# ocrickard/piper-swift

Hardware: AMD Instinct MI355X
Metric: audio-sec/wall-sec (RTF^-1) with ms/utterance, Piper VITS en_GB-medium geometry, scale-bench factor (higher is better)
Workload: dtype f32; 1 GPU; medium factor=8: 112 ids, 336 frames, 86016 samples (3.901 s audio) per utterance, 1 utterance per step per GPU; factor=8, phoneme_count=112, frames=336, samples=86016, parallelism=utterance-replicas x1 (one-shot RCCL weight broadcast)

## Files before the change

### piper-swift_amd/csrc/conv.h

```cpp
#pragma once
#include "common.h"

namespace ph {

enum Prologue : int {
  PRO_NONE = 0,
  PRO_LRELU = 1,
  PRO_AVG3_LRELU = 2,
  PRO_LN = 3,
};

enum Epilogue : int {
  EPI_STORE = 0,
  EPI_RELU = 1,
  EPI_TANH = 2,
  EPI_RSUB = 3,
  EPI_WN_RES_SKIP = 4,
  EPI_WN_SKIP_LAST = 5,
  EPI_CONVT = 6,
  EPI_MRF_MEAN = 7,
};

struct ConvArgs {
  const float* x = nullptr;
// ... 1 lines not shown
  const float* x3 = nullptr;
  const float* w = nullptr;
  const float* w16 = nullptr;
  const float* w8 = nullptr;
  const float* w16g = nullptr;
  const float* bias = nullptr;
  const float* res = nullptr;
  const float* skip = nullptr;
  float* y = nullptr;
  float* y2 = nullptr;
  int N = 1, Cin = 0, Cout = 0, K = 1, dil = 1, padL = 0, Lin = 0, Lout = 0;
  int stride = 1, groups = 1;
  int64_t x_batch_stride = 0;
  int64_t y_batch_stride = 0;
  int64_t y2_batch_stride = 0;
  int in_ch_base = 0, in_ch_sign = 1;
  int out_ch_base = 0, out_ch_sign = 1;
  int y_len = 0;
  int prologue = PRO_NONE;
  float alpha = 0.0f;
  int epilogue = EPI_STORE;
  int gate = 0;
  unsigned long long* trace = nullptr;
  int wn_c = 0;
  int ct_stride = 0, ct_padL = 0, ct_Lout = 0;
  int ct_shift = -1;
  const float* mrf_a = nullptr;
  const float* mrf_b = nullptr;
  float alpha2 = 0.0f;
  const int* len_ptr = nullptr;
  int len_mul = 1;
  float* stats_out = nullptr;
  const float* ln_stats = nullptr;
  const float* ln_gamma = nullptr;
  const float* ln_beta = nullptr;
  float* ln_out = nullptr;
  float ln_eps = 1e-5f;
  int ln_self = 0;
};

size_t packed_conv_floats(int Cout, int Cin, int K, int tm = 32);
size_t packed_convt_floats(int Cin, int Cout, int K, int s, int tm = 32);
int pack_conv_weights(hipStream_t s, const float* w, int Cout, int Cin, int K, float* packed, int tm = 32);
int pack_convt_weights(hipStream_t s, const float* w, int Cin, int Cout, int K, int stride, float* packed, int tm = 32);
int pack_conv_weights_gate16(hipStream_t s, const float* w, int Cout, int Cin, int K, float* packed);
size_t packed_conv_rows8_floats(int Cout, int Cin, int K);
int pack_conv_weights_rows8(hipStream_t s, const float* w, int Cout, int Cin, int K, float* packed);
int conv_pick_tile(piper_hip_ctx* ctx, int Cout, int Lout, int N, int gate);

bool conv_mfma_eligible(int Cout, int Cin, int K, int stride, int groups);
int launch_conv_mfma(piper_hip_ctx* ctx, hipStream_t s, const ConvArgs& a);
int try_launch_conv_lean(piper_hip_ctx* ctx, hipStream_t s, const ConvArgs& a);
bool conv_lean_ln_self_ok(piper_hip_ctx* ctx, int Cin, int Cout, int K, int padL, int L, int N);
int try_launch_conv_short(piper_hip_ctx* ctx, hipStream_t s, const ConvArgs& a);
int launch_conv_direct(piper_hip_ctx* ctx, hipStream_t s, const ConvArgs& a);
int launch_convt_direct(piper_hip_ctx* ctx, hipStream_t s, const float* x, const float* w, const float* bias, float* y, int N,
                        int Cin, int Lin, int Cout, int K, int stride, int dil, int padL, int Lout, int groups);

inline double conv_flops(int Cout, int Cin_per_g, int K, int64_t Lout) { return 2.0 * Cout * (double)Lout * Cin_per_g * K; }

}
```

### piper-swift_amd/csrc/conv_lean.hip

```cpp
#include "conv.h"

namespace ph {
namespace {

typedef float f32x4 __attribute__((ext_vector_type(4)));

struct LeanArgs {
  const float *x, *w, *bias, *res, *skip;
  float *y, *y2;
  const int* len_ptr;
  int len_mul, Lin, Lout, Cout, y_len, nsteps, wn_c;
  int x_row_bytes;
  int x_base_bytes;
  int q_stride;
  int kk_sign;
  int out_ch_base, out_ch_sign;
  int x_batch_bytes;
  long long x_bs, y_bs, y2_bs;
};

__device__ __forceinline__ float bload(__amdgpu_buffer_rsrc_t r, int voff, int soff) {
  return __builtin_bit_cast(float, __builtin_amdgcn_raw_buffer_load_b32(r, voff, soff, 0));
}

// ... 13 lines not shown
  const int soff0 = a.x_base_bytes + wave * NQ * a.q_stride;
  float av[NQ], bv[NQ];
#pragma unroll
  for (int i = 0; i < NQ; i++) av[i] = wa[i * 64];
  {
    const int voff = vrow + min(ch * 16 + j, a.Lin - 1) * 4;
#pragma unroll
    for (int i = 0; i < NQ; i++) bv[i] = bload(rx, voff, soff0 + i * a.q_stride);
  }
  const int row = 16 * mt + 4 * kk + wave;
  const float bias = (wave < 4 && a.bias) ? a.bias[min(row, a.Cout - 1)] : 0.0f;
  for (int it = 0;; it++) {
    const int t0 = ch * 16;
    const int nxt = ch + (int)gridDim.y;
    const bool more = nxt < nch && nxt * 16 < lim;
    f32x4 acc = {0.0f, 0.0f, 0.0f, 0.0f};
#pragma unroll
    for (int i = 0; i < NQ; i++) acc = __builtin_amdgcn_mfma_f32_16x16x4f32(av[i], bv[i], acc, 0, 0, 0);
    if (more) {
      const int voff = vrow + min(nxt * 16 + j, a.Lin - 1) * 4;
#pragma unroll
      for (int i = 0; i < NQ; i++) bv[i] = bload(rx, voff, soff0 + i * a.q_stride);
    }
    float* red = red_all + (it & 1) * (8 * 4 * 64);
#pragma unroll
    for (int r = 0; r < 4; r++) red[(wave * 4 + r) * 64 + lane] = acc[r];
    __syncthreads();
    if (wave < 4) {
      const int col = t0 + j;
      float v = bias;
      float part[8];
#pragma unroll
      for (int s = 0; s < 8; s++) part[s] = red[(s * 4 + wave) * 64 + lane];
#pragma unroll
      for (int s = 0; s < 8; s++) v += part[s];
      if (row < a.Cout && col < a.Lout) {
        if constexpr (MODE == EPI_STORE) {
          const long long idx = (long long)n * a.y_bs + (a.out_ch_base + a.out_ch_sign * row) * a.y_len + col;
          a.y[idx] = a.res ? v + a.res[idx] : v;
        } else if constexpr (MODE == EPI_RSUB) {
          const long long idx = (long long)n * a.y_bs + (a.out_ch_base + a.out_ch_sign * row) * a.y_len + col;
          a.y[idx] = a.res[idx] - v;
        } else if constexpr (MODE == EPI_WN_RES_SKIP) {
          if (row < a.wn_c) {
            const long long idx = (long long)n * a.y_bs + row * a.y_len + col;
            a.y[idx] = a.res[idx] + v;
          } else {
            const long long idx = (long long)n * a.y2_bs + (row - a.wn_c) * a.y_len + col;
            a.y2[idx] = (a.skip ? a.skip[idx] : 0.0f) + v;
          }
        } else {
          const long long idx = (long long)n * a.y2_bs + row * a.y_len + col;
          a.y2[idx] = (a.skip ? a.skip[idx] : 0.0f) + v;
        }
      }
    }
    if (!more) break;
    ch = nxt;
  }
}

struct GateArgs {
  const float *x, *w, *bias;
  float* y;
  const int* len_ptr;
  int len_mul, Lin, Lout, rows_out, y_len, nsteps, pad, x_batch_bytes;
  long long x_bs, y_bs;
};

template <int K, int NQ>
__global__ __launch_bounds__(512) void conv_gate_kernel(const GateArgs a, const int nch) {
  constexpr int W = 16 + K - 1, PITCH = (W + 3) & ~3, ROWS = 4 * NQ, NS = NQ * K;
  constexpr int NLB = (ROWS + 15) / 16;
  constexpr int OOB = 0x7fffffff;
  static_assert(K - 1 <= 4, "halo piece is four columns wide");
  __shared__ float xs_all[8 * ROWS * PITCH];
  __shared__ float red_all[2 * 8 * 4 * 64];
  const int lane = threadIdx.x & 63;
  const int wave = __builtin_amdgcn_readfirstlane((int)(threadIdx.x >> 6));
  const int mt = blockIdx.x, n = blockIdx.z;
  const int Lv = a.len_ptr ? min(a.len_ptr[n] * a.len_mul, a.Lin) : a.Lin;
  int ch = blockIdx.y;
  if (ch * 16 >= Lv) return;
  const int j = lane & 15, kk = lane >> 4;
  const __amdgpu_buffer_rsrc_t rx = __builtin_amdgcn_make_buffer_rsrc((void*)(a.x + (long long)n * a.x_bs), 0, a.x_batch_bytes, 0x00020000);
  const float* wa = a.w + (((long long)mt * a.nsteps + wave * NS) << 6) + lane;
  float av[NS];
#pragma unroll
  for (int s = 0; s < NS; s++) av[s] = wa[s * 64];
  const int rB = lane >> 2, cB = 16 + (lane & 3);
  const int sbase = wave * ROWS * a.Lin * 4;
  float xa[NQ], xb[NLB];
  auto request = [&](int t0) {
    const int posA = t0 - a.pad + j;
    const int voffA = (posA >= 0 && posA < Lv) ? (kk * a.Lin + posA) * 4 : OOB;
    const int posB = t0 - a.pad + cB;
    const int voffB = ((lane & 3) < K - 1 && posB >= 0 && posB < Lv) ? (rB * a.Lin + posB) * 4 : OOB;
#pragma unroll
    for (int i = 0; i < NQ; i++) xa[i] = bload(rx, voffA, sbase + i * 16 * a.Lin);
#pragma unroll
    for (int i = 0; i < NLB; i++) xb[i] = bload(rx, (rB + 16 * i < ROWS) ? voffB : OOB, sbase + i * 64 * a.Lin);
  };
  request(ch * 16);
  float* xs = xs_all + wave * (ROWS * PITCH);
  const float* xw = xs + kk * PITCH + j;
  const int i8 = 4 * kk + wave;
// ... 395 lines not shown
  }
  if (c.K == 3 && c.w8 && c.Cin == 768 && c.prologue == PRO_NONE && c.epilogue == EPI_STORE && !c.stats_out && !c.gate && c.dil == 1 && c.padL == 1 &&
      c.Lin == c.Lout && c.in_ch_sign == 1 && c.in_ch_base == 0 && c.out_ch_sign == 1 && c.out_ch_base == 0 && c.N <= 65535) {
    const int mt8 = (int)ceil_div(c.Cout, 8), nch = (int)ceil_div(c.Lout, 16);
    if ((int64_t)mt8 * nch * c.N <= 2 * (int64_t)ctx->num_cus && nch <= 65535 && c.x_batch_stride * 4 < 0x7fffffffLL) {
      LeanArgs a;
      a.x = c.x; a.w = c.w8; a.bias = c.bias; a.res = c.res; a.skip = nullptr; a.y = c.y; a.y2 = nullptr;
      a.len_ptr = c.len_ptr; a.len_mul = c.len_mul;
      a.Lin = c.Lin; a.Lout = c.Lout; a.Cout = c.Cout; a.y_len = c.y_len; a.wn_c = 0; a.nsteps = (c.Cin / 4) * c.K;
      a.x_row_bytes = c.Lin * 4; a.kk_sign = 1; a.x_base_bytes = 0; a.q_stride = 16 * c.Lin; a.out_ch_base = 0; a.out_ch_sign = 1;
      a.x_batch_bytes = (int)(c.x_batch_stride * 4); a.x_bs = c.x_batch_stride; a.y_bs = c.y_batch_stride; a.y2_bs = 0;
      const int w_bytes = mt8 * a.nsteps * 128;
      constexpr int NQ = 24;
      const size_t lds = (size_t)(8 * 4 * 64 + 8 * (4 * NQ) * 20) * sizeof(float);
      static bool configured[kMaxDevices] = {};
      if (lds_optin_needed(configured))
        (void)hipFuncSetAttribute((const void*)conv_k3_r8_kernel<NQ>, hipFuncAttributeMaxDynamicSharedMemorySize, 160 * 1024);
      hipLaunchKernelGGL((conv_k3_r8_kernel<NQ>), dim3((unsigned)mt8, (unsigned)nch, (unsigned)c.N), dim3(512), lds, s, a, w_bytes);
      hipError_t e = hipGetLastError();
      if (e != hipSuccess) PH_FAIL(PIPER_HIP_ERR_LAUNCH, "conv_lean (8-row tiles) launch failed: %s", hipGetErrorString(e));
      return 1;
    }
  }
  if (c.K != 1 || c.prologue != PRO_NONE || c.stats_out || !c.w16) return 0;
  if (c.epilogue != EPI_STORE && c.epilogue != EPI_RSUB && c.epilogue != EPI_WN_RES_SKIP && c.epilogue != EPI_WN_SKIP_LAST) return 0;
  if ((c.epilogue == EPI_RSUB || c.epilogue == EPI_WN_RES_SKIP) && !c.res) return 0;
  if (c.Cin % 32 || c.padL != 0 || c.Lin != c.Lout || c.N > 65535 || c.Lout < 1) return 0;
  const int NQ = c.Cin / 32;
  if (NQ != 3 && NQ != 6) return 0;
  if (c.in_ch_sign != 1 && c.in_ch_sign != -1) return 0;
  const int mtiles = (int)ceil_div(c.Cout, 16), nchunks = (int)ceil_div(c.Lout, 16);
  if ((int64_t)mtiles * nchunks * c.N > 64 * (int64_t)ctx->num_cus) return 0;
  if (c.x_batch_stride * 4 >= 0x7fffffffLL) return 0;
  LeanArgs a;
  a.x = c.x; a.w = c.w16; a.bias = c.bias; a.res = c.res; a.skip = c.skip; a.y = c.y; a.y2 = c.y2;
  a.len_ptr = c.len_ptr; a.len_mul = c.len_mul;
  a.Lin = c.Lin; a.Lout = c.Lout; a.Cout = c.Cout; a.y_len = c.y_len; a.wn_c = c.wn_c;
  a.nsteps = c.Cin / 4;
  a.x_row_bytes = c.Lin * 4;
  a.kk_sign = c.in_ch_sign;
  a.x_base_bytes = (c.in_ch_sign > 0 ? c.in_ch_base : c.in_ch_base - 3) * c.Lin * 4;
  a.q_stride = c.in_ch_sign * 16 * c.Lin;
  a.out_ch_base = c.out_ch_base; a.out_ch_sign = c.out_ch_sign;
  a.x_batch_bytes = (int)(c.x_batch_stride * 4);
  a.x_bs = c.x_batch_stride; a.y_bs = c.y_batch_stride; a.y2_bs = c.y2_batch_stride;
  const dim3 grid((unsigned)mtiles, (unsigned)chunk_groups(ctx, mtiles, nchunks, c.N), (unsigned)c.N);
  const bool ok = NQ == 3 ? launch_lean_nq<3>(s, grid, a, c.epilogue, nchunks) : launch_lean_nq<6>(s, grid, a, c.epilogue, nchunks);
  if (!ok) return 0;
  hipError_t e = hipGetLastError();
  if (e != hipSuccess) PH_FAIL(PIPER_HIP_ERR_LAUNCH, "conv_lean launch failed: %s", hipGetErrorString(e));
  return 1;
}

}
namespace ph { namespace { PH_WARM(conv_lean, (conv_k1_kernel<6, 0>)); } }
```

### piper-swift_amd/csrc/voice.hip

```cpp
#include <algorithm>
#include <cmath>
#include <cstdlib>
#include <chrono>
#include <functional>
#include <memory>

#include "../../include/piper_hip_voice_layout.h"
#include "conv.h"
#include "conv_bf16.h"
#include "conv_win.h"
#include "rng.h"

namespace ph {
int validate_config(const piper_hip_voice_config* c);
int launch_rel_attention(piper_hip_ctx* ctx, hipStream_t s, const float* q, const float* k, const float* v, const float* ek,
                         const float* ev, float* out, int N, int H, int d, int T, int w, int64_t in_batch_stride,
                         int64_t out_batch_stride, const int* len_ptr);
int rel_attention_split_parts(piper_hip_ctx* ctx, int N, int H, int d, int T, int w);
int launch_rel_attention_split(piper_hip_ctx* ctx, hipStream_t s, const float* q, const float* k, const float* v, const float* ek,
                               const float* ev, float* out, int N, int H, int d, int T, int w, int64_t in_batch_stride,
                               int64_t out_batch_stride, const int* len_ptr, int nsplit, float* part_o, float* part_ml);
size_t dp_scalars_bytes(int n);
void dp_scalars_fill(void* host, int i, float noise_w, float length_scale, unsigned gen, unsigned seed);
bool flow_seam_eligible(int H, int half);
// ... 174 lines not shown
  hipEvent_t ev_in = nullptr;
  float* stats = nullptr;
  std::vector<void*> owned;
  int64_t* ids = nullptr;
  int32_t* frame2id = nullptr;
  float* noise = nullptr;
  float* noise_scale = nullptr;
  unsigned* rng = nullptr;
  float* audio = nullptr;
  int64_t n_samples = 0;
  std::vector<Step> steps;
  struct Tap {
    const float* p;
    int C, row, unit;
    size_t batch_stride;
  };
  std::map<std::string, Tap> taps;
  hipGraph_t graph = nullptr;
  hipGraphExec_t exec = nullptr;
  bool timed = false;
  bool parallel = false;
  float* zin = nullptr;
  const float* z_out = nullptr;
  hipGraph_t front_graph = nullptr;
  hipGraphExec_t front_exec = nullptr;
  int st_chunk = 0, st_next = -1, st_halo = 0;
  int bs_n = 0;
  std::vector<int> bs_next;
  std::vector<uint8_t> bs_dropped;
  int* bs_desc = nullptr;
  float* bs_pack = nullptr;
  size_t bs_pack_cap = 0;
};

}

struct piper_hip_voice {
  piper_hip_ctx* ctx = nullptr;
  piper_hip_voice_config cfg{};
  float* blob = nullptr;
  float* packed = nullptr;
  size_t blob_floats = 0, packed_floats = 0;
  std::map<std::string, piper_tensor_desc> index;
  struct EncLayer {
    ConvW qkv, o, f1, f2;
    const float *ek, *ev, *g1, *b1, *g2, *b2;
    float* qkv_bias;
  };
  std::vector<EncLayer> enc;
  ConvW proj;
  struct Coupling {
    ConvW pre, post;
    std::vector<ConvW> in, rs;
  };
  std::vector<Coupling> flows;
  ConvW conv_pre, conv_post;
  struct DdsLayer {
    const float *dw_w, *dw_b, *g1, *b1, *g2, *b2;
    ConvW pw;
  };
  struct DpBlock {
    int flow = 0;
    ConvW pre, proj;
    std::vector<DdsLayer> dds;
  };
  std::vector<DpBlock> dp;
  const float *dp_m = nullptr, *dp_logs = nullptr;
  struct Stage {
    ConvW up;
    int Cin, Cout, K, stride, pad;
    std::vector<std::vector<ConvW>> rb;
  };
  std::vector<Stage> stages;
  struct ConvWB {
    const uint16_t* w = nullptr;
    const float* bias = nullptr;
    int Cout = 0, Cin = 0, K = 0;
  };
  int precision = PIPER_HIP_PRECISION_F32;
  ConvWB conv_pre_b;
  std::vector<ConvWB> up_b;
  std::vector<std::vector<std::vector<ConvWB>>> rb_b;
  std::vector<void*> owned;
  std::vector<std::unique_ptr<Slot>> plans;
  std::vector<StreamSet> free_sets;
  double last_build_ms[6] = {0, 0, 0, 0, 0, 0};
  size_t plan_cache_max = 128, plan_cache_bytes = (size_t)24 << 30;
  struct Staging {
    int64_t* h_ids = nullptr; int32_t* h_f2i = nullptr; int* h_lens = nullptr; float* h_audio = nullptr;
    size_t cap_t = 0, cap_f = 0, cap_lens = 0, audio_cap = 0;
    char* h_misc = nullptr; float* h_dpn = nullptr; int32_t* h_res = nullptr;
    size_t cap_misc = 0, cap_dpn = 0, cap_res = 0;
    float* h_noise = nullptr;
    size_t cap_noise = 0;
    int* h_desc = nullptr;
    size_t cap_desc = 0;
    std::vector<hipEvent_t> chunk_ev;
  } staging[kMaxSlots];
  Slot* attached[kMaxSlots] = {};
  Slot* attached_dp[kMaxSlots] = {};
  uint64_t use_clock = 0;
  int hop = 1;
};

namespace {

// ... 62 lines not shown
  const piper_hip_voice_config& c = v->cfg;
  const int H = c.hidden, I = c.inter;
  char nm[128];
  v->enc.clear(); v->flows.clear(); v->stages.clear();
  for (int l = 0; l < c.n_layers; l++) {
    piper_hip_voice::EncLayer L{};
    L.qkv_bias = qkv_bias ? (*qkv_bias)[l] : nullptr;
    L.qkv.Cout = 3 * H; L.qkv.Cin = H; L.qkv.K = 1; L.qkv.mfma = true;
    float* p = pk.take(3 * packed_conv_floats(H, H, 1));
    float* p16 = pk.take(3 * packed_conv_floats(H, H, 1, 16));
    L.qkv.w = p;
    L.qkv.w16 = p16;
    if (!dry) {
      static const char* qkv[3] = {"conv_q", "conv_k", "conv_v"};
      for (int j = 0; j < 3; j++) {
        snprintf(nm, sizeof nm, "enc_p.encoder.attn_layers.%d.%s", l, qkv[j]);
        pack_conv_weights(pk.s, tensor(v, std::string(nm) + ".weight"), H, H, 1, p + j * packed_conv_floats(H, H, 1));
        pack_conv_weights(pk.s, tensor(v, std::string(nm) + ".weight"), H, H, 1, p16 + j * packed_conv_floats(H, H, 1, 16), 16);
        PH_HIP(hipMemcpyAsync(L.qkv_bias + j * H, tensor(v, std::string(nm) + ".bias"), H * sizeof(float),
                              hipMemcpyDeviceToDevice, pk.s), PIPER_HIP_ERR_LAUNCH);
      }
      L.qkv.bias = L.qkv_bias;
    }
    snprintf(nm, sizeof nm, "enc_p.encoder.attn_layers.%d.conv_o", l);
    L.o = make_conv(pk, dry, nm, H, H, 1);
    snprintf(nm, sizeof nm, "enc_p.encoder.ffn_layers.%d.conv_1", l);
    L.f1 = make_conv(pk, dry, nm, c.ffn, H, c.ffn_kernel);
    snprintf(nm, sizeof nm, "enc_p.encoder.ffn_layers.%d.conv_2", l);
    L.f2 = make_conv(pk, dry, nm, H, c.ffn, c.ffn_kernel, true, false, false, true);
    if (!dry) {
      snprintf(nm, sizeof nm, "enc_p.encoder.attn_layers.%d.emb_rel_k", l); L.ek = tensor(v, nm);
      snprintf(nm, sizeof nm, "enc_p.encoder.attn_layers.%d.emb_rel_v", l); L.ev = tensor(v, nm);
      snprintf(nm, sizeof nm, "enc_p.encoder.norm_layers_1.%d.gamma", l); L.g1 = tensor(v, nm);
      snprintf(nm, sizeof nm, "enc_p.encoder.norm_layers_1.%d.beta", l); L.b1 = tensor(v, nm);
      snprintf(nm, sizeof nm, "enc_p.encoder.norm_layers_2.%d.gamma", l); L.g2 = tensor(v, nm);
      snprintf(nm, sizeof nm, "enc_p.encoder.norm_layers_2.%d.beta", l); L.b2 = tensor(v, nm);
    }
    v->enc.push_back(L);
  }
  v->proj = make_conv(pk, dry, "enc_p.proj", 2 * I, H, 1);
  for (int f = 0; f < c.n_flows; f++) {
    piper_hip_voice::Coupling C;
    snprintf(nm, sizeof nm, "flow.flows.%d.pre", 2 * f);
    C.pre = make_conv(pk, dry, nm, H, I / 2, 1);
    for (int i = 0; i < c.wn_layers; i++) {
      snprintf(nm, sizeof nm, "flow.flows.%d.enc.in_layers.%d", 2 * f, i);
      C.in.push_back(make_conv(pk, dry, nm, 2 * H, H, c.wn_kernel, true, false, true));
      snprintf(nm, sizeof nm, "flow.flows.%d.enc.res_skip_layers.%d", 2 * f, i);
      C.rs.push_back(make_conv(pk, dry, nm, (i + 1 < c.wn_layers) ? 2 * H : H, H, 1));
    }
    snprintf(nm, sizeof nm, "flow.flows.%d.post", 2 * f);
    C.post = make_conv(pk, dry, nm, I / 2, H, 1);
    v->flows.push_back(C);
  }
  v->conv_pre = make_conv(pk, dry, "dec.conv_pre", c.up_initial, I, 7);
  int ch = c.up_initial;
  for (int u = 0; u < c.n_ups; u++) {
    piper_hip_voice::Stage S;
    S.Cin = ch; S.Cout = ch / 2; S.K = c.up_kernels[u]; S.stride = c.up_rates[u]; S.pad = (S.K - S.stride) / 2;
    const int J = (S.K + S.stride - 1) / S.stride;
    S.up.Cout = S.Cout * S.stride; S.up.Cin = S.Cin; S.up.K = J; S.up.mfma = true;
    float* p = pk.take(packed_convt_floats(S.Cin, S.Cout, S.K, S.stride));
    float* p16 = pk.take(packed_convt_floats(S.Cin, S.Cout, S.K, S.stride, 16));
    S.up.w = p;
    S.up.w16 = p16;
    const bool ct_win = convt_win_eligible(S.Cin, S.Cout, S.K, S.stride, S.pad, 4);
    float* p4 = ct_win ? pk.take(packed_convt_win_floats(S.Cin, S.Cout, S.K, S.stride)) : nullptr;
    S.up.w4 = ct_win ? p4 : nullptr;
    const bool ct_pipe = convt_pipe_eligible(S.Cin, S.Cout, S.K, S.stride, S.pad, 4);
    float* p5 = ct_pipe ? pk.take(packed_convt_pipe_floats(S.Cin, S.Cout, S.K, S.stride)) : nullptr;
    S.up.w5 = p5;
    if (!dry) {
      snprintf(nm, sizeof nm, "dec.ups.%d", u);
      if (ct_win) pack_convt_weights_win(pk.s, tensor(v, std::string(nm) + ".weight"), S.Cin, S.Cout, S.K, S.stride, S.pad, p4);
      if (ct_pipe) pack_convt_weights_pipe(pk.s, tensor(v, std::string(nm) + ".weight"), S.Cin, S.Cout, S.K, S.stride, S.pad, p5);
      pack_convt_weights(pk.s, tensor(v, std::string(nm) + ".weight"), S.Cin, S.Cout, S.K, S.stride, p);
      pack_convt_weights(pk.s, tensor(v, std::string(nm) + ".weight"), S.Cin, S.Cout, S.K, S.stride, p16, 16);
      S.up.bias = tensor(v, std::string(nm) + ".bias");
    }
    ch /= 2;
    for (int j = 0; j < c.n_rb; j++) {
      std::vector<ConvW> convs;
      const int rb = u * c.n_rb + j;
      for (int d = 0; d < c.rb_n_dil; d++) {
        if (c.resblock_type == 1) {
          snprintf(nm, sizeof nm, "dec.resblocks.%d.convs1.%d", rb, d);
          convs.push_back(make_conv(pk, dry, nm, ch, ch, c.rb_kernels[j], true, true));
          snprintf(nm, sizeof nm, "dec.resblocks.%d.convs2.%d", rb, d);
          convs.push_back(make_conv(pk, dry, nm, ch, ch, c.rb_kernels[j], true, true));
        } else {
          snprintf(nm, sizeof nm, "dec.resblocks.%d.convs.%d", rb, d);
          convs.push_back(make_conv(pk, dry, nm, ch, ch, c.rb_kernels[j], true, true));
        }
      }
      S.rb.push_back(convs);
    }
    v->stages.push_back(S);
  }
  v->conv_post = make_conv(pk, dry, "dec.conv_post", 1, ch, 7, false);
  v->dp.clear();
  if (c.dp_present) {
    auto dds_of = [&](const std::string& base) {
      std::vector<piper_hip_voice::DdsLayer> out;
      for (int i = 0; i < c.dp_dds_layers; i++) {
        piper_hip_voice::DdsLayer d{};
        const std::string sep = base + ".convs.convs_sep." + std::to_string(i), n1 = base + ".convs.norms_1." + std::to_string(i),
// ... 821 lines not shown
        a.res = x; a.stats_out = ln_self ? nullptr : st1;
        b.conv(p + (ln_self ? "o_add" : "o_add_stats"), L.o, a, T);
        ln1_pending = true;
      } else {
        b.conv(p + "o", L.o, b.plain(att, y, H, H, T, lensT), T);
        add_ln(p + "add_ln1", x, y, L.g1, L.b1, x1);
      }
    }
    {
      ConvArgs a = b.plain(ln1_pending ? y : x1, ff, H, c.ffn, T, lensT);
      a.padL = (kf - 1) / 2;
      if (ln1_pending) a = with_ln(a, st1, L.g1, L.b1, x1);
      a.epilogue = EPI_RELU;
      b.conv(p + (ln1_pending ? "ln1_ffn1_relu" : "ffn1_relu"), L.f1, a, T);
      ConvArgs a2 = b.plain(ff, y, c.ffn, H, T, lensT);
      a2.padL = (kf - 1) / 2;
      if (ln_ok) { a2.res = x1; a2.stats_out = ln_self ? nullptr : st2; }
      b.conv(p + (ln_self ? "ffn2_add" : ln_ok ? "ffn2_add_stats" : "ffn2"), L.f2, a2, T);
    }
    if (!ln_ok) add_ln(p + "add_ln2", x1, y, L.g2, L.b2, x);
  }
  b.tap("enc_out", x, H, T, 0);
  const bool ln2_pending = ln_ok && c.n_layers > 0;
  if (ln2_pending && for_predictor) add_ln("enc.ln2_final", y, nullptr, v->enc[c.n_layers - 1].g2, v->enc[c.n_layers - 1].b2, x);
  if (ln2_pending && !for_predictor)
    b.conv("enc.ln2_proj", v->proj, with_ln(b.plain(y, stats, H, 2 * I, T, lensT), st2, v->enc[c.n_layers - 1].g2, v->enc[c.n_layers - 1].b2, x), T);
  else
    b.conv("enc.proj", v->proj, b.plain(x, stats, H, 2 * I, T, lensT), T);
  return PIPER_HIP_OK;
}

const float* build_flow(Builder& b, const FrontBuffers& fb) {
  piper_hip_voice* v = b.v;
  Slot& s = b.s;
  const int T = b.T, F = b.F, NB = b.NB;
  const int* lensF = b.lensF;
  const piper_hip_voice_config& c = v->cfg;
  const int H = c.hidden, I = c.inter;
  float *stats = fb.stats, *zp = fb.zp, *zflip = fb.zflip, *zp_tap = fb.zp_tap, *h = fb.h, *acts = fb.acts, *skip = fb.skip;
  {
    const int32_t* f2i = s.frame2id;
    const float* nz = s.noise;
    const float* nsd = s.noise_scale;
    const unsigned* rngd = s.rng;
    b.step("expand_noise", "", NB * 2.0 * 2.0 * F * (double)I * T, NB * 2.0 * 4.0 * ((double)F * T + (double)T * I + (double)F * I), [=](hipStream_t q) {
      const int grid = (int)std::min<int64_t>(ceil_div((int64_t)I * F, kBlock), 4096);
      hipLaunchKernelGGL(expand_noise_kernel, dim3(grid, NB), dim3(kBlock), 0, q, stats, f2i, nz, zp, zp_tap, I, T, F, nsd, rngd, lensF);
      return PIPER_HIP_OK;
    });
  }
  b.tap("z_p", zp_tap, I, F, 1);
  bool flipped = false;
  const int half = I / 2;
  for (int f = c.n_flows - 1; f >= 0; f--) {
    flipped = !flipped;
    const auto& C = v->flows[f];
    const std::string p = "flow" + std::to_string(f) + ".";
    static const bool no_seam = getenv("PIPER_HIP_NO_FLOW_SEAM") != nullptr;
    auto seam_ok = [&](const piper_hip_voice::Coupling& A, const piper_hip_voice::Coupling& B) {
      return !no_seam && I == 2 * half && flow_seam_eligible(H, half) && A.post.w16 && B.pre.w16 && A.post.bias && B.pre.bias && A.post.K == 1 && B.pre.K == 1 &&
             A.post.Cin == H && A.post.Cout == half && B.pre.Cin == half && B.pre.Cout == H;
    };
    const bool pre_done = f + 1 < c.n_flows && seam_ok(v->flows[f + 1], C);
    if (!pre_done) {
      ConvArgs a = b.plain(zp, h, I, H, F, lensF);
      a.in_ch_base = flipped ? I - 1 : 0;
      a.in_ch_sign = flipped ? -1 : 1;
      b.conv(p + "pre", C.pre, a, F);
    }
    for (int i = 0; i < c.wn_layers; i++) {
      const bool last = i + 1 == c.wn_layers;
      ConvArgs a = b.plain(h, acts, H, H, F, lensF);
      a.padL = (c.wn_kernel - 1) / 2;
      a.gate = 1;
      b.conv(p + "wn" + std::to_string(i) + ".in_gate", C.in[i], a, F);
      ConvArgs a2 = b.plain(acts, h, H, H, F, lensF);
      a2.y2 = skip; a2.y2_batch_stride = (int64_t)H * F;
      a2.skip = i == 0 ? nullptr : skip;
      if (last) a2.epilogue = EPI_WN_SKIP_LAST;
      else { a2.epilogue = EPI_WN_RES_SKIP; a2.wn_c = H; a2.res = h; }
      b.conv(p + "wn" + std::to_string(i) + ".res_skip", C.rs[i], a2, F);
    }
    if (f > 0 && seam_ok(C, v->flows[f - 1])) {
      const auto& Nx = v->flows[f - 1];
      const float *p16 = C.post.w16, *pb = C.post.bias, *q16 = Nx.pre.w16, *qb = Nx.pre.bias;
      const int ps = (int)(packed_conv_floats(half, H, 1, 16) / ((size_t)ceil_div(half, 16) * 64));
      const int qs = (int)(packed_conv_floats(H, half, 1, 16) / ((size_t)ceil_div(H, 16) * 64));
      const int ob = flipped ? I - 1 - half : half, os = flipped ? -1 : 1;
      b.step(p + "post_sub_flip_pre" + std::to_string(f - 1), "conv_mfma", NB * (conv_flops(half, H, 1, F) + conv_flops(H, half, 1, F)),
             NB * 4.0 * ((double)H * F + 2.0 * half * F + (double)H * F + 2.0 * half * H),
             [=](hipStream_t q) { return launch_flow_seam(q, skip, zp, h, p16, pb, q16, qb, NB, H, half, F, ps, qs, ob, os, lensF); });
    } else {
      ConvArgs a = b.plain(skip, zp, H, I, F, lensF);
      a.epilogue = EPI_RSUB;
      a.res = zp;
      a.out_ch_base = flipped ? I - 1 - half : half;
      a.out_ch_sign = flipped ? -1 : 1;
      b.conv(p + "post_sub", C.post, a, F);
    }
  }
  if (!flipped) return zp;
  b.step("flow.final_flip", "", 0, 0, [=](hipStream_t q) {
    const int grid = (int)std::min<int64_t>(ceil_div((int64_t)I * F, kBlock), 4096);
    hipLaunchKernelGGL(flip_channels_kernel, dim3(grid, NB), dim3(kBlock), 0, q, zp, zflip, I, F);
    return PIPER_HIP_OK;
  });
  return zflip;
}

int build_duration_predictor(Builder& b, const float* x) {
  piper_hip_voice* v = b.v;
  Slot& s = b.s;
  Arena& ar = b.ar;
  const int T = b.T, NB = b.NB;
  const piper_hip_voice_config& c = v->cfg;
  piper_hip_ctx* ctx = v->ctx;
  const int H = c.hidden, nbins = c.dp_bins, K = c.dp_kernel;
  const size_t B = (size_t)NB;
  if (!c.dp_present || v->dp.empty()) PH_FAIL(PIPER_HIP_ERR_UNSUPPORTED, "voice has no duration predictor (dp_present = 0): supply durations");
  if (!dds_layer_eligible(H, K)) PH_FAIL(PIPER_HIP_ERR_UNSUPPORTED, "duration predictor: hidden %d / kernel %d not covered", H, K);
  float* a0 = ar.f32(B * H * T);
  float* a1 = ar.f32(B * H * T);
  float* cond = ar.f32(B * H * T);
  float* hsp = ar.f32(B * (size_t)(3 * nbins - 1) * T);
  float* z = ar.f32(B * 2 * T);
  float* logw = ar.f32(B * T);
  s.dp_noise = ar.f32(B * 2 * T);
  s.dp_scalars = ar.raw(dp_scalars_bytes(NB));
  s.dp_dur = (int32_t*)ar.raw(B * T * sizeof(int32_t));
  if (ar.rc) return ar.rc;
  const int* lensT = b.lensT;
  auto conv_k1 = [&](const std::string& name, const ConvW& w, const float* in, int64_t in_bs, float* out, const float* res) {
    ConvArgs a;
    a.x = in; a.y = out; a.N = NB; a.Lin = T; a.Lout = T; a.x_batch_stride = in_bs; a.y_batch_stride = (int64_t)w.Cout * T; a.y_len = T;
    a.len_ptr = lensT; a.res = res;
    b.conv(name, w, a, T);
  };
  auto dds_stack = [&](const std::string& name, const std::vector<piper_hip_voice::DdsLayer>& layers, float* cur, float* other) {
    int dil = 1;
    for (size_t i = 0; i < layers.size(); i++) {
      const auto& L = layers[i];
      const float *src = cur, *dw_w = L.dw_w, *dw_b = L.dw_b, *g1 = L.g1, *b1 = L.b1, *pw = L.pw.w16, *pwb = L.pw.bias, *g2 = L.g2, *b2 = L.b2;
      float* dst = other;
      const int steps = (int)(packed_conv_floats(H, H, 1, 16) / ((size_t)ceil_div(H, 16) * 64));
      const int d2 = dil;
      b.step(name + ".dds" + std::to_string(i), "dds_layer", NB * (conv_flops(H, H, 1, T) + conv_flops(H, 1, K, T)), NB * 4.0 * (2.0 * H * T + (double)H * H),
             [=](hipStream_t q) { return launch_dds_layer(ctx, q, src, dw_w, dw_b, g1, b1, pw, pwb, g2, b2, dst, NB, H, T, K, d2, steps, lensT, 1e-5f); });
      std::swap(cur, other);
      dil *= K;
    }
    return cur;
  };
  conv_k1("dp.pre", v->dp[0].pre, x, (int64_t)H * T, a0, nullptr);
  float* r = dds_stack("dp", v->dp[0].dds, a0, a1);
  conv_k1("dp.proj", v->dp[0].proj, r, (int64_t)H * T, cond, nullptr);
  const float* nz = s.dp_noise;
  const void* sc = s.dp_scalars;
  b.step("dp.init_latent", "", 0, 0, [=](hipStream_t q) { return launch_dp_init(q, nz, sc, z, NB, T, lensT); });
  for (size_t bi = 1; bi < v->dp.size(); bi++) {
    const auto& Bk = v->dp[bi];
// ... 1538 lines not shown
```

Measured before the change: 5376 audio-sec/wall-sec.

## Fold last WN res_skip, post and next pre into one flow-tail kernel

Precomputes, at load time and in double precision, a combined weight image that merges the last WaveNet res_skip 1x1 conv with the coupling's post conv and the next flow's pre conv. At inference a single MFMA kernel reads acts, skip and z and writes both the updated z half and the next flow's h. This replaces two launches per flow and skips the intermediate skip/h round trips through memory. In exchange it adds a bigger fused GEMM (K=2H+half), ping-pongs z buffers, and introduces a rounding change from the folded f32 weights.

Result: faster. 5580 audio-sec/wall-sec (median of 6 runs) (+3.8%).

```diff
diff --git a/piper-swift_amd/csrc/conv.h b/piper-swift_amd/csrc/conv.h
--- a/piper-swift_amd/csrc/conv.h
+++ b/piper-swift_amd/csrc/conv.h
@@ -77,6 +77,24 @@
 int launch_conv_mfma(piper_hip_ctx* ctx, hipStream_t s, const ConvArgs& a);
 int try_launch_conv_lean(piper_hip_ctx* ctx, hipStream_t s, const ConvArgs& a);
 bool conv_lean_ln_self_ok(piper_hip_ctx* ctx, int Cin, int Cout, int K, int padL, int L, int N);
+struct FlowTailArgs {
+  const float *acts = nullptr, *skip = nullptr;
+  const float* zin = nullptr;
+  float* zout = nullptr;
+  float* h = nullptr;
+  const float *w = nullptr, *bias = nullptr;
+  const int* len_ptr = nullptr;
+  int N = 1, H = 0, half = 0, F = 0, seam = 0;
+  int out_ch_base = 0, out_ch_sign = 1;
+};
+bool flow_tail_shape_ok(int H, int half);
+bool flow_tail_plan_ok(piper_hip_ctx* ctx, int H, int half, int F, int N);
+inline int flow_tail_steps(int H, int half, int seam) { return (2 * H + (seam ? half : 0)) / 4; }
+inline size_t flow_tail_image_floats(int H, int half, int seam) { return (size_t)((half + (seam ? H : 0)) / 16) * flow_tail_steps(H, half, seam) * 64; }
+inline size_t flow_tail_scratch_doubles(int H, int half) { return (size_t)half * (H + 1) + (size_t)H * H; }
+int fold_flow_tail(hipStream_t s, const float* w_rs, const float* b_rs, const float* w_post, const float* b_post, const float* w_pre, const float* b_pre,
+                   int H, int half, int x1_sign, double* scratch, float* image, float* bias);
+int launch_flow_tail(piper_hip_ctx* ctx, hipStream_t s, const FlowTailArgs& t);
 int try_launch_conv_short(piper_hip_ctx* ctx, hipStream_t s, const ConvArgs& a);
 int launch_conv_direct(piper_hip_ctx* ctx, hipStream_t s, const ConvArgs& a);
 int launch_convt_direct(piper_hip_ctx* ctx, hipStream_t s, const float* x, const float* w, const float* bias, float* y, int N,
diff --git a/piper-swift_amd/csrc/conv_lean.hip b/piper-swift_amd/csrc/conv_lean.hip
--- a/piper-swift_amd/csrc/conv_lean.hip
+++ b/piper-swift_amd/csrc/conv_lean.hip
@@ -89,6 +89,85 @@
         } else {
           const long long idx = (long long)n * a.y2_bs + row * a.y_len + col;
           a.y2[idx] = (a.skip ? a.skip[idx] : 0.0f) + v;
+        }
+      }
+    }
+    if (!more) break;
+    ch = nxt;
+  }
+}
+
+struct TailArgs {
+  const float *acts, *skip, *zin, *w, *bias;
+  float *zout, *h;
+  const int* len_ptr;
+  int L, half, rows, nsteps;
+  int x1_base_bytes;
+  int out_ch_base, out_ch_sign;
+  int hs_batch_bytes, z_batch_bytes;
+  long long hs_bs, z_bs;
+};
+
+template <int NX, int NS, int NA>
+__global__ __launch_bounds__(512) void conv_k1_tail_kernel(const TailArgs a, const int nch) {
+  constexpr int NT = NX + NS + NA;
+  __shared__ float red_all[2 * 8 * 4 * 64];
+  const int lane = threadIdx.x & 63;
+  const int wave = __builtin_amdgcn_readfirstlane((int)(threadIdx.x >> 6));
+  const int mt = blockIdx.x, n = blockIdx.z;
+  const int lim = a.len_ptr ? min(a.len_ptr[n], a.L) : a.L;
+  int ch = blockIdx.y;
+  if (ch * 16 >= lim) return;
+  const int j = lane & 15, kk = lane >> 4;
+  const __amdgpu_buffer_rsrc_t ra = __builtin_amdgcn_make_buffer_rsrc((void*)(a.acts + (long long)n * a.hs_bs), 0, a.hs_batch_bytes, 0x00020000);
+  const __amdgpu_buffer_rsrc_t rs = __builtin_amdgcn_make_buffer_rsrc((void*)(a.skip + (long long)n * a.hs_bs), 0, a.hs_batch_bytes, 0x00020000);
+  const __amdgpu_buffer_rsrc_t rz = __builtin_amdgcn_make_buffer_rsrc((void*)(a.zin + (long long)n * a.z_bs), 0, a.z_batch_bytes, 0x00020000);
+  const float* wa = a.w + (((long long)mt * a.nsteps + wave * NT) << 6) + lane;
+  const int q_stride = 16 * a.L;
+  const int vrow = kk * a.L * 4;
+  const int sx = a.x1_base_bytes + wave * NX * q_stride, ss = wave * NS * q_stride, sa = wave * NA * q_stride;
+  float av[NT], bv[NT];
+#pragma unroll
+  for (int i = 0; i < NT; i++) av[i] = wa[i * 64];
+  auto request = [&](int c16) {
+    const int voff = vrow + min(c16 + j, a.L - 1) * 4;
+#pragma unroll
+    for (int i = 0; i < NX; i++) bv[i] = bload(rz, voff, sx + i * q_stride);
+#pragma unroll
+    for (int i = 0; i < NS; i++) bv[NX + i] = bload(rs, voff, ss + i * q_stride);
+#pragma unroll
+    for (int i = 0; i < NA; i++) bv[NX + NS + i] = bload(ra, voff, sa + i * q_stride);
+  };
+  request(ch * 16);
+  const int row = 16 * mt + 4 * kk + wave;
+  const float bias = wave < 4 ? a.bias[min(row, a.rows - 1)] : 0.0f;
+  const bool to_z = 16 * mt < a.half;
+  for (int it = 0;; it++) {
+    const int t0 = ch * 16;
+    const int nxt = ch + (int)gridDim.y;
+    const bool more = nxt < nch && nxt * 16 < lim;
+    f32x4 acc = {0.0f, 0.0f, 0.0f, 0.0f};
+#pragma unroll
+    for (int i = 0; i < NT; i++) acc = __builtin_amdgcn_mfma_f32_16x16x4f32(av[i], bv[i], acc, 0, 0, 0);
+    if (more) request(nxt * 16);
+    float* red = red_all + (it & 1) * (8 * 4 * 64);
+#pragma unroll
+    for (int r = 0; r < 4; r++) red[(wave * 4 + r) * 64 + lane] = acc[r];
+    __syncthreads();
+    if (wave < 4) {
+      const int col = t0 + j;
+      float v = bias;
+      float part[8];
+#pragma unroll
+      for (int s = 0; s < 8; s++) part[s] = red[(s * 4 + wave) * 64 + lane];
+#pragma unroll
+      for (int s = 0; s < 8; s++) v += part[s];
+      if (row < a.rows && col < a.L) {
+        if (to_z) {
+          const long long idx = (long long)n * a.z_bs + (long long)(a.out_ch_base + a.out_ch_sign * row) * a.L + col;
+          a.zout[idx] = a.zin[idx] - v;
+        } else {
+          a.h[(long long)n * a.hs_bs + (long long)(row - a.half) * a.L + col] = v;
         }
       }
     }
@@ -590,5 +669,34 @@
   return 1;
 }
 
+bool flow_tail_shape_ok(int H, int half) { return H == 192 && half == 96; }
+
+bool flow_tail_plan_ok(piper_hip_ctx* ctx, int H, int half, int F, int N) {
+  static const bool off = getenv("PIPER_HIP_NO_LEAN") != nullptr;
+  if (off || !flow_tail_shape_ok(H, half) || F < 1 || N < 1 || N > 65535) return false;
+  const int64_t tiles = ceil_div(half + H, 16) * ceil_div(F, 16) * (int64_t)N;
+  return tiles <= 64 * (int64_t)ctx->num_cus && (int64_t)std::max(H, 2 * half) * F * 4 < 0x7fffffffLL;
+}
+
+int launch_flow_tail(piper_hip_ctx* ctx, hipStream_t s, const FlowTailArgs& t) {
+  if (!flow_tail_plan_ok(ctx, t.H, t.half, t.F, t.N) || !t.w || !t.bias || !t.acts || !t.skip || !t.zin || !t.zout || (t.seam && (!t.h || t.zin == t.zout)))
+    PH_FAIL(PIPER_HIP_ERR_UNSUPPORTED, "flow_tail: H=%d half=%d F=%d N=%d not covered", t.H, t.half, t.F, t.N);
+  TailArgs a;
+  a.acts = t.acts; a.skip = t.skip; a.zin = t.zin; a.w = t.w; a.bias = t.bias; a.zout = t.zout; a.h = t.h; a.len_ptr = t.len_ptr;
+  a.L = t.F; a.half = t.half; a.rows = t.seam ? t.half + t.H : t.half;
+  a.nsteps = flow_tail_steps(t.H, t.half, t.seam);
+  a.x1_base_bytes = (t.out_ch_sign > 0 ? t.out_ch_base : t.out_ch_base - (t.half - 1)) * t.F * 4;
+  a.out_ch_base = t.out_ch_base; a.out_ch_sign = t.out_ch_sign;
+  a.hs_bs = (long long)t.H * t.F; a.z_bs = (long long)2 * t.half * t.F;
+  a.hs_batch_bytes = (int)(a.hs_bs * 4); a.z_batch_bytes = (int)(a.z_bs * 4);
+  const int mtiles = a.rows / 16, nchunks = (int)ceil_div(t.F, 16);
+  const dim3 grid((unsigned)mtiles, (unsigned)chunk_groups(ctx, mtiles, nchunks, t.N), (unsigned)t.N);
+  if (t.seam) hipLaunchKernelGGL((conv_k1_tail_kernel<3, 6, 6>), grid, dim3(512), 0, s, a, nchunks);
+  else hipLaunchKernelGGL((conv_k1_tail_kernel<0, 6, 6>), grid, dim3(512), 0, s, a, nchunks);
+  hipError_t e = hipGetLastError();
+  if (e != hipSuccess) PH_FAIL(PIPER_HIP_ERR_LAUNCH, "flow_tail launch failed: %s", hipGetErrorString(e));
+  return PIPER_HIP_OK;
+}
+
 }
 namespace ph { namespace { PH_WARM(conv_lean, (conv_k1_kernel<6, 0>)); } }
diff --git a/piper-swift_amd/csrc/flow_fold.hip b/piper-swift_amd/csrc/flow_fold.hip
--- /dev/null
+++ b/piper-swift_amd/csrc/flow_fold.hip
@@ -0,0 +1,91 @@
+#include "conv.h"
+
+namespace ph {
+namespace {
+
+constexpr int kFoldBlock = 256;
+
+__global__ __launch_bounds__(kFoldBlock) void fold_a1_kernel(const float* __restrict__ w_post, const float* __restrict__ b_post, const float* __restrict__ w_rs,
+                                                             const float* __restrict__ b_rs, double* __restrict__ a1, int H, int half) {
+  const int idx = blockIdx.x * kFoldBlock + threadIdx.x;
+  if (idx >= half * (H + 1)) return;
+  const int r = idx / (H + 1), c = idx % (H + 1);
+  double acc = 0.0;
+  if (c < H) {
+    for (int k = 0; k < H; k++) acc += (double)w_post[r * H + k] * (double)w_rs[k * H + c];
+  } else {
+    for (int k = 0; k < H; k++) acc += (double)w_post[r * H + k] * (double)(b_rs ? b_rs[k] : 0.0f);
+    acc += (double)(b_post ? b_post[r] : 0.0f);
+  }
+  a1[idx] = acc;
+}
+
+__global__ __launch_bounds__(kFoldBlock) void fold_pw_kernel(const float* __restrict__ w_pre, const float* __restrict__ w_post, double* __restrict__ pw, int H, int half) {
+  const int idx = blockIdx.x * kFoldBlock + threadIdx.x;
+  if (idx >= H * H) return;
+  const int o = idx / H, k = idx % H;
+  double acc = 0.0;
+  for (int r = 0; r < half; r++) acc += (double)w_pre[o * half + (half - 1 - r)] * (double)w_post[r * H + k];
+  pw[idx] = acc;
+}
+
+__global__ __launch_bounds__(kFoldBlock) void fold_image_kernel(const float* __restrict__ w_rs, const float* __restrict__ w_post, const float* __restrict__ w_pre,
+                                                                const float* __restrict__ b_pre, const double* __restrict__ a1, const double* __restrict__ pw,
+                                                                float* __restrict__ image, float* __restrict__ bias, int H, int half, int seam, int x1_sign) {
+  const int rows = half + (seam ? H : 0);
+  const int NX = seam ? half / 32 : 0, NS = H / 32, NA = H / 32, NT = NX + NS + NA, nsteps = 8 * NT;
+  const int idx = blockIdx.x * kFoldBlock + threadIdx.x;
+  if (idx < rows) {
+    double b;
+    if (idx < half) b = a1[idx * (H + 1) + H];
+    else {
+      const int o = idx - half;
+      b = (double)(b_pre ? b_pre[o] : 0.0f);
+      for (int r = 0; r < half; r++) b -= (double)w_pre[o * half + (half - 1 - r)] * a1[r * (H + 1) + H];
+    }
+    bias[idx] = (float)b;
+  }
+  if (idx >= (rows / 16) * nsteps * 64) return;
+  const int lane = idx & 63, step = (idx >> 6) % nsteps, mt = (idx >> 6) / nsteps;
+  const int row = 16 * mt + (lane & 15), kq = lane >> 4;
+  const int wave = step / NT, i = step % NT;
+  double v;
+  if (i < NX) {
+    const int p = 4 * (wave * NX + i) + kq;
+    const int r = x1_sign > 0 ? p : half - 1 - p;
+    v = row < half ? 0.0 : (double)w_pre[(row - half) * half + (half - 1 - r)];
+  } else if (i < NX + NS) {
+    const int c = 4 * (wave * NS + i - NX) + kq;
+    v = row < half ? (double)w_post[row * H + c] : -pw[(row - half) * H + c];
+  } else {
+    const int c = 4 * (wave * NA + i - NX - NS) + kq;
+    if (row < half) v = a1[row * (H + 1) + c];
+    else {
+      const int o = row - half;
+      v = 0.0;
+      for (int k = 0; k < H; k++) v -= pw[o * H + k] * (double)w_rs[k * H + c];
+    }
+  }
+  image[idx] = (float)v;
+}
+
+}
+
+int fold_flow_tail(hipStream_t s, const float* w_rs, const float* b_rs, const float* w_post, const float* b_post, const float* w_pre, const float* b_pre,
+                   int H, int half, int x1_sign, double* scratch, float* image, float* bias) {
+  const int seam = w_pre != nullptr;
+  if (H % 32 || half % 32 || !w_rs || !w_post || !scratch || !image || !bias) PH_FAIL(PIPER_HIP_ERR_ARG, "fold_flow_tail: H=%d half=%d", H, half);
+  double* a1 = scratch;
+  double* pw = scratch + (size_t)half * (H + 1);
+  hipLaunchKernelGGL(fold_a1_kernel, dim3((unsigned)ceil_div(half * (H + 1), kFoldBlock)), dim3(kFoldBlock), 0, s, w_post, b_post, w_rs, b_rs, a1, H, half);
+  if (seam) hipLaunchKernelGGL(fold_pw_kernel, dim3((unsigned)ceil_div(H * H, kFoldBlock)), dim3(kFoldBlock), 0, s, w_pre, w_post, pw, H, half);
+  const size_t n = flow_tail_image_floats(H, half, seam);
+  hipLaunchKernelGGL(fold_image_kernel, dim3((unsigned)ceil_div((int64_t)n, kFoldBlock)), dim3(kFoldBlock), 0, s, w_rs, w_post, w_pre, b_pre, a1, pw, image, bias, H,
+                     half, seam, x1_sign);
+  hipError_t e = hipGetLastError();
+  if (e != hipSuccess) PH_FAIL(PIPER_HIP_ERR_LAUNCH, "fold_flow_tail launch failed: %s", hipGetErrorString(e));
+  return PIPER_HIP_OK;
+}
+
+}
+namespace ph { namespace { PH_WARM(flow_fold, fold_a1_kernel); } }
diff --git a/piper-swift_amd/csrc/voice.hip b/piper-swift_amd/csrc/voice.hip
--- a/piper-swift_amd/csrc/voice.hip
+++ b/piper-swift_amd/csrc/voice.hip
@@ -250,6 +250,7 @@
   struct Coupling {
     ConvW pre, post;
     std::vector<ConvW> in, rs;
+    const float *tail_w = nullptr, *tail_b = nullptr;
   };
   std::vector<Coupling> flows;
   ConvW conv_pre, conv_post;
@@ -418,6 +419,27 @@
     snprintf(nm, sizeof nm, "flow.flows.%d.post", 2 * f);
     C.post = make_conv(pk, dry, nm, I / 2, H, 1);
     v->flows.push_back(C);
+  }
+  if (flow_tail_shape_ok(H, I / 2) && I % 2 == 0 && c.wn_layers >= 2 && c.n_flows >= 1) {
+    const int half = I / 2;
+    double* scratch = (double*)pk.take(2 * flow_tail_scratch_doubles(H, half));
+    for (int f = 0; f < c.n_flows; f++) {
+      auto& C = v->flows[f];
+      const int seam = f > 0;
+      float* img = pk.take(flow_tail_image_floats(H, half, seam));
+      float* tb = pk.take((size_t)half + (seam ? H : 0));
+      if (dry) continue;
+      auto raw = [&](const char* what, int g) {
+        snprintf(nm, sizeof nm, "flow.flows.%d.%s", 2 * g, what);
+        return std::string(nm);
+      };
+      const std::string rs = raw("enc.res_skip_layers.", f) + std::to_string(c.wn_layers - 1), post = raw("post", f), pre = raw("pre", std::max(f - 1, 0));
+      const int rc = fold_flow_tail(pk.s, tensor(v, rs + ".weight"), tensor(v, rs + ".bias"), tensor(v, post + ".weight"), tensor(v, post + ".bias"),
+                                    seam ? tensor(v, pre + ".weight") : nullptr, seam ? tensor(v, pre + ".bias") : nullptr, H, half,
+                                    (c.n_flows - f) % 2 ? -1 : 1, scratch, img, tb);
+      if (rc) return rc;
+      C.tail_w = img; C.tail_b = tb;
+    }
   }
   v->conv_pre = make_conv(pk, dry, "dec.conv_pre", c.up_initial, I, 7);
   int ch = c.up_initial;
@@ -1345,16 +1367,21 @@
   b.tap("z_p", zp_tap, I, F, 1);
   bool flipped = false;
   const int half = I / 2;
+  static const bool no_seam = getenv("PIPER_HIP_NO_FLOW_SEAM") != nullptr;
+  auto seam_ok = [&](const piper_hip_voice::Coupling& A, const piper_hip_voice::Coupling& B) {
+    return !no_seam && I == 2 * half && flow_seam_eligible(H, half) && A.post.w16 && B.pre.w16 && A.post.bias && B.pre.bias && A.post.K == 1 && B.pre.K == 1 &&
+           A.post.Cin == H && A.post.Cout == half && B.pre.Cin == half && B.pre.Cout == H;
+  };
+  static const bool no_fold = getenv("PIPER_HIP_NO_FLOW_FOLD") != nullptr;
+  bool fold = !no_fold && c.wn_layers >= 2 && flow_tail_plan_ok(v->ctx, H, half, F, NB);
+  for (int f = 0; f < c.n_flows && fold; f++)
+    fold = v->flows[f].tail_w && v->flows[f].tail_b && (f == 0 || seam_ok(v->flows[f], v->flows[f - 1]));
+  float* zloc[2] = {zp, zp};
   for (int f = c.n_flows - 1; f >= 0; f--) {
     flipped = !flipped;
     const auto& C = v->flows[f];
     const std::string p = "flow" + std::to_string(f) + ".";
-    static const bool no_seam = getenv("PIPER_HIP_NO_FLOW_SEAM") != nullptr;
-    auto seam_ok = [&](const piper_hip_voice::Coupling& A, const piper_hip_voice::Coupling& B) {
-      return !no_seam && I == 2 * half && flow_seam_eligible(H, half) && A.post.w16 && B.pre.w16 && A.post.bias && B.pre.bias && A.post.K == 1 && B.pre.K == 1 &&
-             A.post.Cin == H && A.post.Cout == half && B.pre.Cin == half && B.pre.Cout == H;
-    };
-    const bool pre_done = f + 1 < c.n_flows && seam_ok(v->flows[f + 1], C);
+    const bool pre_done = f + 1 < c.n_flows && (fold || seam_ok(v->flows[f + 1], C));
     if (!pre_done) {
       ConvArgs a = b.plain(zp, h, I, H, F, lensF);
       a.in_ch_base = flipped ? I - 1 : 0;
@@ -1367,6 +1394,7 @@
       a.padL = (c.wn_kernel - 1) / 2;
       a.gate = 1;
       b.conv(p + "wn" + std::to_string(i) + ".in_gate", C.in[i], a, F);
+      if (last && fold) break;
       ConvArgs a2 = b.plain(acts, h, H, H, F, lensF);
       a2.y2 = skip; a2.y2_batch_stride = (int64_t)H * F;
       a2.skip = i == 0 ? nullptr : skip;
@@ -1374,31 +1402,45 @@
       else { a2.epilogue = EPI_WN_RES_SKIP; a2.wn_c = H; a2.res = h; }
       b.conv(p + "wn" + std::to_string(i) + ".res_skip", C.rs[i], a2, F);
     }
-    if (f > 0 && seam_ok(C, v->flows[f - 1])) {
+    const int ob = flipped ? I - 1 - half : half, os = flipped ? -1 : 1;
+    const double seam_flops = NB * (conv_flops(half, H, 1, F) + conv_flops(H, half, 1, F));
+    const double seam_bytes = NB * 4.0 * ((double)H * F + 2.0 * half * F + (double)H * F + 2.0 * half * H);
+    if (fold) {
+      const int xh = flipped ? 0 : 1;
+      FlowTailArgs t;
+      t.acts = acts; t.skip = skip; t.zin = zloc[xh]; t.h = h; t.w = C.tail_w; t.bias = C.tail_b; t.len_ptr = lensF;
+      t.N = NB; t.H = H; t.half = half; t.F = F; t.seam = f > 0; t.out_ch_base = ob; t.out_ch_sign = os;
+      t.zout = f > 0 ? (zloc[xh] == zp ? zflip : zp) : zloc[1 - xh];
+      zloc[xh] = t.zout;
+      piper_hip_ctx* ctx = v->ctx;
+      const std::string rs = p + "wn" + std::to_string(c.wn_layers - 1) + ".res_skip_";
+      const double rs_flops = NB * conv_flops(H, H, 1, F), rs_bytes = NB * conv_bytes(H, H, 1, F);
+      if (f > 0) b.step(rs + "post_sub_flip_pre" + std::to_string(f - 1), "conv_mfma", rs_flops + seam_flops, rs_bytes + seam_bytes, [=](hipStream_t q) { return launch_flow_tail(ctx, q, t); });
+      else b.step(rs + "post_sub", "conv_mfma", rs_flops + NB * conv_flops(half, H, 1, F), rs_bytes + NB * conv_bytes(H, half, 1, F), [=](hipStream_t q) { return launch_flow_tail(ctx, q, t); });
+    } else if (f > 0 && seam_ok(C, v->flows[f - 1])) {
       const auto& Nx = v->flows[f - 1];
       const float *p16 = C.post.w16, *pb = C.post.bias, *q16 = Nx.pre.w16, *qb = Nx.pre.bias;
       const int ps = (int)(packed_conv_floats(half, H, 1, 16) / ((size_t)ceil_div(half, 16) * 64));
       const int qs = (int)(packed_conv_floats(H, half, 1, 16) / ((size_t)ceil_div(H, 16) * 64));
-      const int ob = flipped ? I - 1 - half : half, os = flipped ? -1 : 1;
-      b.step(p + "post_sub_flip_pre" + std::to_string(f - 1), "conv_mfma", NB * (conv_flops(half, H, 1, F) + conv_flops(H, half, 1, F)),
-             NB * 4.0 * ((double)H * F + 2.0 * half * F + (double)H * F + 2.0 * half * H),
+      b.step(p + "post_sub_flip_pre" + std::to_string(f - 1), "conv_mfma", seam_flops, seam_bytes,
              [=](hipStream_t q) { return launch_flow_seam(q, skip, zp, h, p16, pb, q16, qb, NB, H, half, F, ps, qs, ob, os, lensF); });
     } else {
       ConvArgs a = b.plain(skip, zp, H, I, F, lensF);
       a.epilogue = EPI_RSUB;
       a.res = zp;
-      a.out_ch_base = flipped ? I - 1 - half : half;
-      a.out_ch_sign = flipped ? -1 : 1;
+      a.out_ch_base = ob;
+      a.out_ch_sign = os;
       b.conv(p + "post_sub", C.post, a, F);
     }
   }
-  if (!flipped) return zp;
+  float *z = zloc[0], *zother = z == zp ? zflip : zp;
+  if (!flipped) return z;
   b.step("flow.final_flip", "", 0, 0, [=](hipStream_t q) {
     const int grid = (int)std::min<int64_t>(ceil_div((int64_t)I * F, kBlock), 4096);
-    hipLaunchKernelGGL(flip_channels_kernel, dim3(grid, NB), dim3(kBlock), 0, q, zp, zflip, I, F);
+    hipLaunchKernelGGL(flip_channels_kernel, dim3(grid, NB), dim3(kBlock), 0, q, z, zother, I, F);
     return PIPER_HIP_OK;
   });
-  return zflip;
+  return zother;
 }
 
 int build_duration_predictor(Builder& b, const float* x) {
```
